# denix56/SI-Mamba

Hardware: AMD Instinct MI355X
Metric: point-clouds/sec (fwd+bwd) (higher is better)
Workload: dtype f32; 1 GPU; PointMamba classifier train step (FPS+kNN grouping, encoder, spectral SAST ordering, 12 Mamba blocks d=384 at L=1024, head, AdamW), 1024 pts -> 128 patches; global_batch=64, per_gpu_batch=64, npoints=1024, patches=128, mamba_seq_len=1024, parallelism=dp1, communicator_ranks=1, library_gemm=tuned solution table (si_mamba_amd/tuned/gemm_gfx950.csv)

## Files before the change

### si_mamba_amd/csrc/add_norm.hip

```cpp
#include "common.h"

namespace simamba {

constexpr int kLnThreads = 256;
constexpr int kLnMaxChunks = 8;

struct LnArgs {
  const void* hidden;
  const float* residual;
  const float* rowscale;
  const float* weight;
  const float* bias;
  float* residual_out;
  void* normed;
  float* mean;
  float* rstd;
  const void* dnormed;
  const float* dresidual_out;
  float* dresidual;
  void* dhidden;
  float* dwb_partial;
  const int* hidden_slot;
  const int* normed_slot;
  int hidden_batch, normed_batch;
  int batch, rows_per_batch, dim;
  float eps;
};

template <typename T>
__device__ __forceinline__ float4 ld4(const T* p) {
  const Pack<T, 4> pk = *reinterpret_cast<const Pack<T, 4>*>(p);
  return make_float4(to_f32<T>(pk.v[0]), to_f32<T>(pk.v[1]), to_f32<T>(pk.v[2]), to_f32<T>(pk.v[3]));
}
template <typename T>
__device__ __forceinline__ void st4(T* p, float4 v) {
  Pack<T, 4> pk;
  pk.v[0] = from_f32<T>(v.x); pk.v[1] = from_f32<T>(v.y); pk.v[2] = from_f32<T>(v.z); pk.v[3] = from_f32<T>(v.w);
  *reinterpret_cast<Pack<T, 4>*>(p) = pk;
}

__device__ __forceinline__ int ln_slot(const int* __restrict__ map, int b, int count) {
  if (!map) return b;
  const int s = __builtin_amdgcn_readfirstlane(map[b]);
  return (s >= 0 && s < count) ? s : -1;
}

struct LnRow {
  int b, hs, os;
};
__device__ __forceinline__ LnRow ln_row(const LnArgs& p, int row) {
  LnRow r;
  r.b = __builtin_amdgcn_readfirstlane(row / p.rows_per_batch);
  r.hs = ln_slot(p.hidden_slot, r.b, p.hidden_batch);
  r.os = ln_slot(p.normed_slot, r.b, p.normed_batch);
  return r;
}

template <typename TH, typename TO, int kChunks, bool kRms>
__global__ __launch_bounds__(kLnThreads) void add_ln_fwd_kernel(LnArgs p) {
  const bool slots = p.hidden_slot || p.normed_slot;
  const int lane = threadIdx.x & 63;
  const int wave_global = (blockIdx.x * kLnThreads + threadIdx.x) >> 6;
  const int nwaves = (gridDim.x * kLnThreads) >> 6;
  const int rows = p.batch * p.rows_per_batch;
  const int nch = p.dim >> 2;
  const TH* __restrict__ hg = static_cast<const TH*>(p.hidden);
  TO* __restrict__ og = static_cast<TO*>(p.normed);
  float4 w[kChunks], bs[kChunks];
#pragma unroll
  for (int k = 0; k < kChunks; ++k) {
    const int c = lane + 64 * k;
    w[k] = c < nch ? *reinterpret_cast<const float4*>(p.weight + 4 * c) : make_float4(0, 0, 0, 0);
    bs[k] = (!kRms && c < nch && p.bias) ? *reinterpret_cast<const float4*>(p.bias + 4 * c) : make_float4(0, 0, 0, 0);
  }
  const float inv_dim = 1.f / p.dim;
  LnRow next = (slots && wave_global < rows) ? ln_row(p, wave_global) : LnRow{0, 0, 0};
  for (int row = wave_global; row < rows; row += nwaves) {
    const size_t base = static_cast<size_t>(row) * p.dim;
    const float scale = (p.rowscale && p.residual) ? p.rowscale[row / p.rows_per_batch] : 1.f;
    size_t hbase = base, obase = base;
    bool has_h = true, has_o = true;
    if (slots) {
      const LnRow cur = next;
      const int ahead = row + nwaves;
      next = ln_row(p, ahead < rows ? ahead : row);
      const int r = __builtin_amdgcn_readfirstlane(row) - cur.b * p.rows_per_batch;
      has_h = cur.hs >= 0; has_o = cur.os >= 0;
      hbase = (static_cast<size_t>(has_h ? cur.hs : 0) * p.rows_per_batch + r) * p.dim;
      obase = (static_cast<size_t>(has_o ? cur.os : 0) * p.rows_per_batch + r) * p.dim;
    }
    float4 x[kChunks];
    float sum = 0.f;
#pragma unroll
    for (int k = 0; k < kChunks; ++k) {
      const int c = lane + 64 * k;
      if (c < nch) {
        float4 h;
        if (!has_h) {
          h = *reinterpret_cast<const float4*>(p.residual + base + 4 * c);
        } else {
          h = ld4<TH>(hg + hbase + 4 * c);
          if (p.residual) {
            const float4 r = *reinterpret_cast<const float4*>(p.residual + base + 4 * c);
            h.x = fmaf(h.x, scale, r.x); h.y = fmaf(h.y, scale, r.y);
            h.z = fmaf(h.z, scale, r.z); h.w = fmaf(h.w, scale, r.w);
          }
        }
        if (p.residual_out) *reinterpret_cast<float4*>(p.residual_out + base + 4 * c) = h;
        x[k] = h;
        sum += (h.x + h.y) + (h.z + h.w);
      } else {
        x[k] = make_float4(0, 0, 0, 0);
      }
    }
    if (!has_o) continue;
    const float mean = kRms ? 0.f : wave_allreduce_sum(sum) * inv_dim;
    float sq = 0.f;
#pragma unroll
    for (int k = 0; k < kChunks; ++k) {
      if (lane + 64 * k < nch) {
        const float a = x[k].x - mean, b = x[k].y - mean, c = x[k].z - mean, d = x[k].w - mean;
        sq += (a * a + b * b) + (c * c + d * d);
      }
    }
    const float rstd = rsqrtf(wave_allreduce_sum(sq) * inv_dim + p.eps);
#pragma unroll
    for (int k = 0; k < kChunks; ++k) {
      const int c = lane + 64 * k;
      if (c < nch) {
        float4 y;
        y.x = fmaf((x[k].x - mean) * rstd, w[k].x, bs[k].x);
        y.y = fmaf((x[k].y - mean) * rstd, w[k].y, bs[k].y);
        y.z = fmaf((x[k].z - mean) * rstd, w[k].z, bs[k].z);
        y.w = fmaf((x[k].w - mean) * rstd, w[k].w, bs[k].w);
        st4<TO>(og + obase + 4 * c, y);
      }
    }
    if (lane == 0) {
      if (!kRms) p.mean[row] = mean;
      p.rstd[row] = rstd;
    }
  }
}

template <typename TH, typename TO, int kChunks, bool kRms>
__global__ __launch_bounds__(kLnThreads) void add_ln_bwd_kernel(LnArgs p) {
  const bool slots = p.hidden_slot || p.normed_slot;
  extern __shared__ float sred[];
  const int lane = threadIdx.x & 63;
  const int wave = threadIdx.x >> 6;
  const int wave_global = (blockIdx.x * kLnThreads + threadIdx.x) >> 6;
  const int nwaves = (gridDim.x * kLnThreads) >> 6;
  const int rows = p.batch * p.rows_per_batch;
  const int nch = p.dim >> 2;
  const TO* __restrict__ dyg = static_cast<const TO*>(p.dnormed);
  TH* __restrict__ dhg = static_cast<TH*>(p.dhidden);
  float4 w[kChunks], dw[kChunks], db[kChunks];
#pragma unroll
  for (int k = 0; k < kChunks; ++k) {
    const int c = lane + 64 * k;
    w[k] = c < nch ? *reinterpret_cast<const float4*>(p.weight + 4 * c) : make_float4(0, 0, 0, 0);
    dw[k] = make_float4(0, 0, 0, 0);
    db[k] = make_float4(0, 0, 0, 0);
  }
  const float inv_dim = 1.f / p.dim;
  LnRow next = (slots && wave_global < rows) ? ln_row(p, wave_global) : LnRow{0, 0, 0};
  for (int row = wave_global; row < rows; row += nwaves) {
    const size_t base = static_cast<size_t>(row) * p.dim;
    size_t hbase = base, obase = base;
    bool has_h = true, has_o = true;
    if (slots) {
      const LnRow cur = next;
      const int ahead = row + nwaves;
      next = ln_row(p, ahead < rows ? ahead : row);
      const int r = __builtin_amdgcn_readfirstlane(row) - cur.b * p.rows_per_batch;
      has_h = cur.hs >= 0; has_o = cur.os >= 0;
      hbase = (static_cast<size_t>(has_h ? cur.hs : 0) * p.rows_per_batch + r) * p.dim;
      obase = (static_cast<size_t>(has_o ? cur.os : 0) * p.rows_per_batch + r) * p.dim;
    }
    if (!has_o) {
      const float scale = (p.rowscale && dhg) ? p.rowscale[row / p.rows_per_batch] : 1.f;
#pragma unroll
      for (int k = 0; k < kChunks; ++k) {
        const int c = lane + 64 * k;
        if (c < nch) {
          const float4 dx = p.dresidual_out ? *reinterpret_cast<const float4*>(p.dresidual_out + base + 4 * c)
                                            : make_float4(0, 0, 0, 0);
          if (p.dresidual) *reinterpret_cast<float4*>(p.dresidual + base + 4 * c) = dx;
          if (dhg && has_h)
            st4<TH>(dhg + hbase + 4 * c, make_float4(dx.x * scale, dx.y * scale, dx.z * scale, dx.w * scale));
        }
      }
      continue;
    }
    const float mean = kRms ? 0.f : p.mean[row], rstd = p.rstd[row];
    float4 xh[kChunks], g[kChunks];
    float s1 = 0.f, s2 = 0.f;
#pragma unroll
    for (int k = 0; k < kChunks; ++k) {
      const int c = lane + 64 * k;
      if (c < nch) {
        const float4 x = *reinterpret_cast<const float4*>(p.residual_out + base + 4 * c);
        const float4 dy = ld4<TO>(dyg + obase + 4 * c);
        xh[k] = make_float4((x.x - mean) * rstd, (x.y - mean) * rstd, (x.z - mean) * rstd, (x.w - mean) * rstd);
        g[k] = make_float4(dy.x * w[k].x, dy.y * w[k].y, dy.z * w[k].z, dy.w * w[k].w);
        dw[k].x = fmaf(dy.x, xh[k].x, dw[k].x); dw[k].y = fmaf(dy.y, xh[k].y, dw[k].y);
        dw[k].z = fmaf(dy.z, xh[k].z, dw[k].z); dw[k].w = fmaf(dy.w, xh[k].w, dw[k].w);
        db[k].x += dy.x; db[k].y += dy.y; db[k].z += dy.z; db[k].w += dy.w;
        s1 += (g[k].x + g[k].y) + (g[k].z + g[k].w);
        s2 += (g[k].x * xh[k].x + g[k].y * xh[k].y) + (g[k].z * xh[k].z + g[k].w * xh[k].w);
      } else {
        xh[k] = make_float4(0, 0, 0, 0);
        g[k] = make_float4(0, 0, 0, 0);
      }
    }
    const float c1 = kRms ? 0.f : wave_allreduce_sum(s1) * inv_dim;
    const float c2 = wave_allreduce_sum(s2) * inv_dim;
    const float scale = (p.rowscale && dhg) ? p.rowscale[row / p.rows_per_batch] : 1.f;
#pragma unroll
    for (int k = 0; k < kChunks; ++k) {
      const int c = lane + 64 * k;
      if (c < nch) {
        float4 dx;
        dx.x = (g[k].x - c1 - xh[k].x * c2) * rstd;
        dx.y = (g[k].y - c1 - xh[k].y * c2) * rstd;
        dx.z = (g[k].z - c1 - xh[k].z * c2) * rstd;
        dx.w = (g[k].w - c1 - xh[k].w * c2) * rstd;
        if (p.dresidual_out) {
          const float4 r = *reinterpret_cast<const float4*>(p.dresidual_out + base + 4 * c);
          dx.x += r.x; dx.y += r.y; dx.z += r.z; dx.w += r.w;
        }
        if (p.dresidual) *reinterpret_cast<float4*>(p.dresidual + base + 4 * c) = dx;
        if (dhg && has_h)
          st4<TH>(dhg + hbase + 4 * c, make_float4(dx.x * scale, dx.y * scale, dx.z * scale, dx.w * scale));
      }
    }
  }
  float* mine = sred + wave * 2 * p.dim;
#pragma unroll
  for (int k = 0; k < kChunks; ++k) {
    const int c = lane + 64 * k;
    if (c < nch) {
      *reinterpret_cast<float4*>(mine + 4 * c) = dw[k];
      if (!kRms) *reinterpret_cast<float4*>(mine + p.dim + 4 * c) = db[k];
    }
  }
  __syncthreads();
  float* out = p.dwb_partial + static_cast<size_t>(blockIdx.x) * 2 * p.dim;
  for (int i = threadIdx.x; i < (kRms ? 1 : 2) * p.dim; i += kLnThreads) {
    float v = 0.f;
#pragma unroll
    for (int wv = 0; wv < kLnThreads / 64; ++wv) v += sred[wv * 2 * p.dim + i];
    out[i] = v;
  }
}

static int ln_grid(int rows) {
  int g = (rows + 3) / 4;
  return g < 1 ? 1 : (g > 1024 ? 1024 : g);
}

template <typename TH, typename TO, bool kRms>
static int launch_ln(const LnArgs& a, bool bwd, int grid, hipStream_t s) {
  const int chunks = ((a.dim >> 2) + 63) / 64;
#define SIMAMBA_LN_CASE(K)                                                                                      \
  if (chunks <= K) {                                                                                             \
    if (bwd)                                                                                                     \
      hipLaunchKernelGGL((add_ln_bwd_kernel<TH, TO, K, kRms>), dim3(grid), dim3(kLnThreads),                     \
                         sizeof(float) * (kLnThreads / 64) * 2 * a.dim, s, a);                                   \
    else                                                                                                         \
      hipLaunchKernelGGL((add_ln_fwd_kernel<TH, TO, K, kRms>), dim3(grid), dim3(kLnThreads), 0, s, a);           \
    return static_cast<int>(hipGetLastError());                                                                  \
  }
  SIMAMBA_LN_CASE(1)
  SIMAMBA_LN_CASE(2)
  SIMAMBA_LN_CASE(4)
  SIMAMBA_LN_CASE(8)
#undef SIMAMBA_LN_CASE
  return SIMAMBA_E_SHAPE;
}

template <typename TH, typename TO>
static int launch_ln(const LnArgs& a, bool bwd, bool rms, int grid, hipStream_t s) {
  return rms ? launch_ln<TH, TO, true>(a, bwd, grid, s) : launch_ln<TH, TO, false>(a, bwd, grid, s);
}

static int dispatch_ln(const LnArgs& a, bool bwd, bool rms, int grid, int hidden_dtype, int out_dtype, hipStream_t s) {
  if (hidden_dtype == SIMAMBA_F32 && out_dtype == SIMAMBA_F32) return launch_ln<float, float>(a, bwd, rms, grid, s);
  if (hidden_dtype == SIMAMBA_BF16 && out_dtype == SIMAMBA_BF16)
    return launch_ln<bf16_t, bf16_t>(a, bwd, rms, grid, s);
  if (hidden_dtype == SIMAMBA_F32 && out_dtype == SIMAMBA_BF16) return launch_ln<float, bf16_t>(a, bwd, rms, grid, s);
  if (hidden_dtype == SIMAMBA_BF16 && out_dtype == SIMAMBA_F32) return launch_ln<bf16_t, float>(a, bwd, rms, grid, s);
  return SIMAMBA_E_DTYPE;
}

}

using namespace simamba;

static int check_ln(int batch, int rows_per_batch, int dim) {
  if (batch < 0 || rows_per_batch < 0) return SIMAMBA_E_SHAPE;
  if (dim <= 0 || (dim & 3) || dim > 64 * 4 * kLnMaxChunks) return SIMAMBA_E_SHAPE;
  return SIMAMBA_OK;
}

extern "C" int simamba_add_layer_norm_grid(int batch, int rows_per_batch) {
  const long long rows = static_cast<long long>(batch) * rows_per_batch;
  return ln_grid(rows > 2000000000ll ? 2000000000 : static_cast<int>(rows));
}

static int check_slots(const int* map, int compact_batch, int batch) {
  if (compact_batch < 0 || compact_batch > batch) return SIMAMBA_E_SHAPE;
  if (!map && compact_batch != batch) return SIMAMBA_E_NULLPTR;
  return SIMAMBA_OK;
}

extern "C" int simamba_add_layer_norm_check_slots(const int* slots_host, int batch, int compact_batch) {
  if (batch < 0 || compact_batch < 0 || compact_batch > batch) return SIMAMBA_E_SHAPE;
  if (batch == 0) return SIMAMBA_OK;
  if (!slots_host) return SIMAMBA_E_NULLPTR;
  for (int b = 0; b < batch; ++b) {
    const int s = slots_host[b];
    if (s < -1 || s >= compact_batch) return SIMAMBA_E_SHAPE;
    if (s < 0) continue;
    for (int c = 0; c < b; ++c)
      if (slots_host[c] == s) return SIMAMBA_E_SHAPE;
  }
  return SIMAMBA_OK;
}

extern "C" int simamba_add_layer_norm_fwd_slots(const void* hidden, const float* residual, const float* rowscale,
                                                const float* weight, const float* bias, float* residual_out,
                                                void* normed, float* mean, float* rstd, const int* hidden_slot,
                                                int hidden_batch, const int* normed_slot, int normed_batch, int batch,
                                                int rows_per_batch, int dim, float eps, int hidden_dtype,
                                                int out_dtype, int flags, void* stream) {
  if (flags & ~SIMAMBA_NORM_RMS) return SIMAMBA_E_VARIANT;
  const bool rms = (flags & SIMAMBA_NORM_RMS) != 0;
  if (rms && bias) return SIMAMBA_E_BIAS;
  int rc = check_ln(batch, rows_per_batch, dim);
  if (rc) return rc;
  if (batch == 0 || rows_per_batch == 0) return SIMAMBA_OK;
  if ((rc = check_slots(hidden_slot, hidden_batch, batch))) return rc;
  if ((rc = check_slots(normed_slot, normed_batch, batch))) return rc;
  if ((!hidden && hidden_batch) || !weight || (!normed && normed_batch) || (!mean && !rms) || !rstd)
    return SIMAMBA_E_NULLPTR;
  if (hidden_slot && (!residual || !residual_out)) return SIMAMBA_E_NULLPTR;
  LnArgs a{};
  a.hidden = hidden; a.residual = residual; a.rowscale = rowscale; a.weight = weight; a.bias = bias;
  a.residual_out = residual_out; a.normed = normed; a.mean = mean; a.rstd = rstd;
  a.hidden_slot = hidden_slot; a.normed_slot = normed_slot; a.hidden_batch = hidden_batch; a.normed_batch = normed_batch;
  a.batch = batch; a.rows_per_batch = rows_per_batch; a.dim = dim; a.eps = eps;
  return dispatch_ln(a, false, rms, simamba_add_layer_norm_grid(batch, rows_per_batch), hidden_dtype, out_dtype,
                     static_cast<hipStream_t>(stream));
}

extern "C" int simamba_add_layer_norm_fwd_ex(const void* hidden, const float* residual, const float* rowscale,
                                             const float* weight, const float* bias, float* residual_out, void* normed,
                                             float* mean, float* rstd, int batch, int rows_per_batch, int dim,
                                             float eps, int hidden_dtype, int out_dtype, int flags, void* stream) {
  return simamba_add_layer_norm_fwd_slots(hidden, residual, rowscale, weight, bias, residual_out, normed, mean, rstd,
                                          nullptr, batch, nullptr, batch, batch, rows_per_batch, dim, eps, hidden_dtype,
                                          out_dtype, flags, stream);
}

extern "C" int simamba_add_layer_norm_fwd(const void* hidden, const float* residual, const float* rowscale,
                                          const float* weight, const float* bias, float* residual_out, void* normed,
                                          float* mean, float* rstd, int batch, int rows_per_batch, int dim, float eps,
                                          int hidden_dtype, int out_dtype, void* stream) {
  return simamba_add_layer_norm_fwd_ex(hidden, residual, rowscale, weight, bias, residual_out, normed, mean, rstd,
                                       batch, rows_per_batch, dim, eps, hidden_dtype, out_dtype, 0, stream);
}

extern "C" int simamba_add_layer_norm_bwd_slots(const void* dnormed, const float* dresidual_out,
                                                const float* residual_out, const float* mean, const float* rstd,
                                                const float* weight, const float* rowscale, float* dresidual,
                                                void* dhidden, float* dwb_partial, const int* hidden_slot,
                                                int hidden_batch, const int* normed_slot, int normed_batch, int batch,
                                                int rows_per_batch, int dim, int hidden_dtype, int out_dtype,
                                                int flags, void* stream) {
  if (flags & ~SIMAMBA_NORM_RMS) return SIMAMBA_E_VARIANT;
  const bool rms = (flags & SIMAMBA_NORM_RMS) != 0;
  int rc = check_ln(batch, rows_per_batch, dim);
  if (rc) return rc;
  if (batch == 0 || rows_per_batch == 0) return SIMAMBA_OK;
  if ((rc = check_slots(hidden_slot, hidden_batch, batch))) return rc;
  if ((rc = check_slots(normed_slot, normed_batch, batch))) return rc;
  if (hidden_batch == 0) dhidden = nullptr;
  if ((!dnormed || !residual_out || (!mean && !rms) || !rstd) && normed_batch) return SIMAMBA_E_NULLPTR;
  if (!weight || !dwb_partial || (!dresidual && !dhidden)) return SIMAMBA_E_NULLPTR;
  LnArgs a{};
  a.dnormed = dnormed; a.dresidual_out = dresidual_out; a.residual_out = const_cast<float*>(residual_out);
  a.mean = const_cast<float*>(mean); a.rstd = const_cast<float*>(rstd); a.weight = weight; a.rowscale = rowscale;
  a.dresidual = dresidual; a.dhidden = dhidden; a.dwb_partial = dwb_partial;
  a.hidden_slot = hidden_slot; a.normed_slot = normed_slot; a.hidden_batch = hidden_batch; a.normed_batch = normed_batch;
  a.batch = batch; a.rows_per_batch = rows_per_batch; a.dim = dim;
  return dispatch_ln(a, true, rms, simamba_add_layer_norm_grid(batch, rows_per_batch), hidden_dtype, out_dtype,
                     static_cast<hipStream_t>(stream));
}

extern "C" int simamba_add_layer_norm_bwd_ex(const void* dnormed, const float* dresidual_out,
                                             const float* residual_out, const float* mean, const float* rstd,
                                             const float* weight, const float* rowscale, float* dresidual,
                                             void* dhidden, float* dwb_partial, int batch, int rows_per_batch, int dim,
                                             int hidden_dtype, int out_dtype, int flags, void* stream) {
  return simamba_add_layer_norm_bwd_slots(dnormed, dresidual_out, residual_out, mean, rstd, weight, rowscale, dresidual,
                                          dhidden, dwb_partial, nullptr, batch, nullptr, batch, batch, rows_per_batch,
                                          dim, hidden_dtype, out_dtype, flags, stream);
}

extern "C" int simamba_add_layer_norm_bwd(const void* dnormed, const float* dresidual_out, const float* residual_out,
                                          const float* mean, const float* rstd, const float* weight,
                                          const float* rowscale, float* dresidual, void* dhidden, float* dwb_partial,
                                          int batch, int rows_per_batch, int dim, int hidden_dtype, int out_dtype,
                                          void* stream) {
  return simamba_add_layer_norm_bwd_ex(dnormed, dresidual_out, residual_out, mean, rstd, weight, rowscale, dresidual,
                                       dhidden, dwb_partial, batch, rows_per_batch, dim, hidden_dtype, out_dtype, 0,
                                       stream);
}
```

Before: 1161 point-clouds/s.

## Preload slot maps into lanes and issue row loads unconditionally in add-LN kernels

The per-batch slot maps and rowscales are loaded once per wave into registers and fetched with readlane, instead of scalar global loads on every row. Row loads for hidden, residual, dy and x are issued up front without branches, using clamped offsets and a dummy pointer for absent rows. In the backward kernel the dresidual_out load is hoisted early when there are few chunks. The aim is to overlap memory latency and drop per-row dependent scalar loads, at the cost of higher register pressure and some wasted loads.

```diff
diff --git a/si_mamba_amd/csrc/add_norm.hip b/si_mamba_amd/csrc/add_norm.hip
--- a/si_mamba_amd/csrc/add_norm.hip
+++ b/si_mamba_amd/csrc/add_norm.hip
@@ -28,8 +28,7 @@
 };
 
 template <typename T>
-__device__ __forceinline__ float4 ld4(const T* p) {
-  const Pack<T, 4> pk = *reinterpret_cast<const Pack<T, 4>*>(p);
+__device__ __forceinline__ float4 unpack4(const Pack<T, 4>& pk) {
   return make_float4(to_f32<T>(pk.v[0]), to_f32<T>(pk.v[1]), to_f32<T>(pk.v[2]), to_f32<T>(pk.v[3]));
 }
 template <typename T>
@@ -41,71 +40,120 @@
 
 __device__ __forceinline__ int ln_slot(const int* __restrict__ map, int b, int count) {
   if (!map) return b;
-  const int s = __builtin_amdgcn_readfirstlane(map[b]);
+  const int s = map[b];
   return (s >= 0 && s < count) ? s : -1;
+}
+
+constexpr int kLnMapRegs = 2;
+struct LnSamples {
+  int hs[kLnMapRegs], os[kLnMapRegs];
+  float scale[kLnMapRegs];
+  bool resident;
+};
+__device__ __forceinline__ LnSamples ln_samples(const LnArgs& p, int lane, bool use_scale) {
+  LnSamples m;
+  m.resident = p.batch <= 64 * kLnMapRegs;
+#pragma unroll
+  for (int j = 0; j < kLnMapRegs; ++j) {
+    const int b = lane + 64 * j;
+    const bool in = m.resident && b < p.batch;
+    m.hs[j] = in ? ln_slot(p.hidden_slot, b, p.hidden_batch) : -1;
+    m.os[j] = in ? ln_slot(p.normed_slot, b, p.normed_batch) : -1;
+    m.scale[j] = (in && use_scale) ? p.rowscale[b] : 1.f;
+  }
+  return m;
 }
 
 struct LnRow {
   int b, hs, os;
+  float scale;
 };
-__device__ __forceinline__ LnRow ln_row(const LnArgs& p, int row) {
+__device__ __forceinline__ LnRow ln_row(const LnArgs& p, const LnSamples& m, bool use_scale, int row) {
   LnRow r;
   r.b = __builtin_amdgcn_readfirstlane(row / p.rows_per_batch);
-  r.hs = ln_slot(p.hidden_slot, r.b, p.hidden_batch);
-  r.os = ln_slot(p.normed_slot, r.b, p.normed_batch);
+  if (m.resident) {
+    int hs = m.hs[0], os = m.os[0];
+    float sc = m.scale[0];
+#pragma unroll
+    for (int j = 1; j < kLnMapRegs; ++j)
+      if ((r.b >> 6) == j) { hs = m.hs[j]; os = m.os[j]; sc = m.scale[j]; }
+    r.hs = __builtin_amdgcn_readlane(hs, r.b & 63);
+    r.os = __builtin_amdgcn_readlane(os, r.b & 63);
+    r.scale = __builtin_bit_cast(float, __builtin_amdgcn_readlane(__builtin_bit_cast(int, sc), r.b & 63));
+  } else {
+    r.hs = __builtin_amdgcn_readfirstlane(ln_slot(p.hidden_slot, r.b, p.hidden_batch));
+    r.os = __builtin_amdgcn_readfirstlane(ln_slot(p.normed_slot, r.b, p.normed_batch));
+    r.scale = use_scale ? __builtin_bit_cast(float, __builtin_amdgcn_readfirstlane(
+                              __builtin_bit_cast(int, p.rowscale[r.b])))
+                        : 1.f;
+  }
   return r;
+}
+
+__device__ __forceinline__ void ln_setup_loads_done() {
+  __builtin_amdgcn_s_waitcnt(0x0f70);
 }
 
 template <typename TH, typename TO, int kChunks, bool kRms>
 __global__ __launch_bounds__(kLnThreads) void add_ln_fwd_kernel(LnArgs p) {
-  const bool slots = p.hidden_slot || p.normed_slot;
   const int lane = threadIdx.x & 63;
-  const int wave_global = (blockIdx.x * kLnThreads + threadIdx.x) >> 6;
+  const int wave_global = __builtin_amdgcn_readfirstlane((blockIdx.x * kLnThreads + threadIdx.x) >> 6);
   const int nwaves = (gridDim.x * kLnThreads) >> 6;
   const int rows = p.batch * p.rows_per_batch;
   const int nch = p.dim >> 2;
   const TH* __restrict__ hg = static_cast<const TH*>(p.hidden);
   TO* __restrict__ og = static_cast<TO*>(p.normed);
   float4 w[kChunks], bs[kChunks];
+  int off[kChunks];
+  bool valid[kChunks];
 #pragma unroll
   for (int k = 0; k < kChunks; ++k) {
     const int c = lane + 64 * k;
+    valid[k] = c < nch;
+    off[k] = 4 * (valid[k] ? c : nch - 1);
     w[k] = c < nch ? *reinterpret_cast<const float4*>(p.weight + 4 * c) : make_float4(0, 0, 0, 0);
     bs[k] = (!kRms && c < nch && p.bias) ? *reinterpret_cast<const float4*>(p.bias + 4 * c) : make_float4(0, 0, 0, 0);
   }
   const float inv_dim = 1.f / p.dim;
-  LnRow next = (slots && wave_global < rows) ? ln_row(p, wave_global) : LnRow{0, 0, 0};
+  const bool use_scale = p.rowscale && p.residual;
+  const LnSamples samples = ln_samples(p, lane, use_scale);
+  ln_setup_loads_done();
+  LnRow next = wave_global < rows ? ln_row(p, samples, use_scale, wave_global) : LnRow{0, 0, 0, 1.f};
   for (int row = wave_global; row < rows; row += nwaves) {
+    const LnRow cur = next;
+    const int ahead = row + nwaves;
+    next = ln_row(p, samples, use_scale, ahead < rows ? ahead : row);
     const size_t base = static_cast<size_t>(row) * p.dim;
-    const float scale = (p.rowscale && p.residual) ? p.rowscale[row / p.rows_per_batch] : 1.f;
-    size_t hbase = base, obase = base;
-    bool has_h = true, has_o = true;
-    if (slots) {
-      const LnRow cur = next;
-      const int ahead = row + nwaves;
-      next = ln_row(p, ahead < rows ? ahead : row);
-      const int r = __builtin_amdgcn_readfirstlane(row) - cur.b * p.rows_per_batch;
-      has_h = cur.hs >= 0; has_o = cur.os >= 0;
-      hbase = (static_cast<size_t>(has_h ? cur.hs : 0) * p.rows_per_batch + r) * p.dim;
-      obase = (static_cast<size_t>(has_o ? cur.os : 0) * p.rows_per_batch + r) * p.dim;
+    const int r = row - cur.b * p.rows_per_batch;
+    const bool has_h = cur.hs >= 0, has_o = cur.os >= 0;
+    const float scale = cur.scale;
+    const TH* hrow = has_h ? hg + (static_cast<size_t>(cur.hs) * p.rows_per_batch + r) * p.dim
+                           : reinterpret_cast<const TH*>(p.weight);
+    const size_t obase = (static_cast<size_t>(has_o ? cur.os : 0) * p.rows_per_batch + r) * p.dim;
+    Pack<TH, 4> hraw[kChunks];
+    float4 res[kChunks];
+#pragma unroll
+    for (int k = 0; k < kChunks; ++k) hraw[k] = *reinterpret_cast<const Pack<TH, 4>*>(hrow + off[k]);
+    if (p.residual) {
+#pragma unroll
+      for (int k = 0; k < kChunks; ++k) res[k] = *reinterpret_cast<const float4*>(p.residual + base + off[k]);
     }
     float4 x[kChunks];
     float sum = 0.f;
 #pragma unroll
     for (int k = 0; k < kChunks; ++k) {
       const int c = lane + 64 * k;
-      if (c < nch) {
-        float4 h;
-        if (!has_h) {
-          h = *reinterpret_cast<const float4*>(p.residual + base + 4 * c);
+      float4 h = unpack4<TH>(hraw[k]);
+      if (p.residual) {
+        const float4 rr = res[k];
+        if (has_h) {
+          h.x = fmaf(h.x, scale, rr.x); h.y = fmaf(h.y, scale, rr.y);
+          h.z = fmaf(h.z, scale, rr.z); h.w = fmaf(h.w, scale, rr.w);
         } else {
-          h = ld4<TH>(hg + hbase + 4 * c);
-          if (p.residual) {
-            const float4 r = *reinterpret_cast<const float4*>(p.residual + base + 4 * c);
-            h.x = fmaf(h.x, scale, r.x); h.y = fmaf(h.y, scale, r.y);
-            h.z = fmaf(h.z, scale, r.z); h.w = fmaf(h.w, scale, r.w);
-          }
+          h = rr;
         }
+      }
+      if (valid[k]) {
         if (p.residual_out) *reinterpret_cast<float4*>(p.residual_out + base + 4 * c) = h;
         x[k] = h;
         sum += (h.x + h.y) + (h.z + h.w);
@@ -113,12 +161,11 @@
         x[k] = make_float4(0, 0, 0, 0);
       }
     }
-    if (!has_o) continue;
     const float mean = kRms ? 0.f : wave_allreduce_sum(sum) * inv_dim;
     float sq = 0.f;
 #pragma unroll
     for (int k = 0; k < kChunks; ++k) {
-      if (lane + 64 * k < nch) {
+      if (valid[k]) {
         const float a = x[k].x - mean, b = x[k].y - mean, c = x[k].z - mean, d = x[k].w - mean;
         sq += (a * a + b * b) + (c * c + d * d);
       }
@@ -127,7 +174,7 @@
 #pragma unroll
     for (int k = 0; k < kChunks; ++k) {
       const int c = lane + 64 * k;
-      if (c < nch) {
+      if (valid[k] && has_o) {
         float4 y;
         y.x = fmaf((x[k].x - mean) * rstd, w[k].x, bs[k].x);
         y.y = fmaf((x[k].y - mean) * rstd, w[k].y, bs[k].y);
@@ -136,7 +183,7 @@
         st4<TO>(og + obase + 4 * c, y);
       }
     }
-    if (lane == 0) {
+    if (lane == 0 && has_o) {
       if (!kRms) p.mean[row] = mean;
       p.rstd[row] = rstd;
     }
@@ -145,47 +192,69 @@
 
 template <typename TH, typename TO, int kChunks, bool kRms>
 __global__ __launch_bounds__(kLnThreads) void add_ln_bwd_kernel(LnArgs p) {
-  const bool slots = p.hidden_slot || p.normed_slot;
   extern __shared__ float sred[];
   const int lane = threadIdx.x & 63;
   const int wave = threadIdx.x >> 6;
-  const int wave_global = (blockIdx.x * kLnThreads + threadIdx.x) >> 6;
+  const int wave_global = __builtin_amdgcn_readfirstlane((blockIdx.x * kLnThreads + threadIdx.x) >> 6);
   const int nwaves = (gridDim.x * kLnThreads) >> 6;
   const int rows = p.batch * p.rows_per_batch;
   const int nch = p.dim >> 2;
   const TO* __restrict__ dyg = static_cast<const TO*>(p.dnormed);
   TH* __restrict__ dhg = static_cast<TH*>(p.dhidden);
+  constexpr bool kEarlyRes = kChunks <= 4;
   float4 w[kChunks], dw[kChunks], db[kChunks];
+  int off[kChunks];
+  bool valid[kChunks];
 #pragma unroll
   for (int k = 0; k < kChunks; ++k) {
     const int c = lane + 64 * k;
+    valid[k] = c < nch;
+    off[k] = 4 * (valid[k] ? c : nch - 1);
     w[k] = c < nch ? *reinterpret_cast<const float4*>(p.weight + 4 * c) : make_float4(0, 0, 0, 0);
     dw[k] = make_float4(0, 0, 0, 0);
     db[k] = make_float4(0, 0, 0, 0);
   }
   const float inv_dim = 1.f / p.dim;
-  LnRow next = (slots && wave_global < rows) ? ln_row(p, wave_global) : LnRow{0, 0, 0};
+  const bool use_scale = p.rowscale && dhg;
+  const LnSamples samples = ln_samples(p, lane, use_scale);
+  ln_setup_loads_done();
+  LnRow next = wave_global < rows ? ln_row(p, samples, use_scale, wave_global) : LnRow{0, 0, 0, 1.f};
   for (int row = wave_global; row < rows; row += nwaves) {
+    const LnRow cur = next;
+    const int ahead = row + nwaves;
+    next = ln_row(p, samples, use_scale, ahead < rows ? ahead : row);
     const size_t base = static_cast<size_t>(row) * p.dim;
-    size_t hbase = base, obase = base;
-    bool has_h = true, has_o = true;
-    if (slots) {
-      const LnRow cur = next;
-      const int ahead = row + nwaves;
-      next = ln_row(p, ahead < rows ? ahead : row);
-      const int r = __builtin_amdgcn_readfirstlane(row) - cur.b * p.rows_per_batch;
-      has_h = cur.hs >= 0; has_o = cur.os >= 0;
-      hbase = (static_cast<size_t>(has_h ? cur.hs : 0) * p.rows_per_batch + r) * p.dim;
-      obase = (static_cast<size_t>(has_o ? cur.os : 0) * p.rows_per_batch + r) * p.dim;
+    const int r = row - cur.b * p.rows_per_batch;
+    const bool has_h = cur.hs >= 0, has_o = cur.os >= 0;
+    const float scale = cur.scale;
+    const size_t hbase = (static_cast<size_t>(has_h ? cur.hs : 0) * p.rows_per_batch + r) * p.dim;
+    const float* xrow = has_o ? p.residual_out + base : p.weight;
+    const TO* dyrow = has_o ? dyg + (static_cast<size_t>(cur.os) * p.rows_per_batch + r) * p.dim
+                            : reinterpret_cast<const TO*>(p.weight);
+    const float* mrow = (has_o && !kRms) ? p.mean + row : p.weight;
+    const float* srow = has_o ? p.rstd + row : p.weight;
+    float4 xraw[kChunks], res[kChunks];
+    Pack<TO, 4> dyraw[kChunks];
+#pragma unroll
+    for (int k = 0; k < kChunks; ++k) {
+      xraw[k] = *reinterpret_cast<const float4*>(xrow + off[k]);
+      dyraw[k] = *reinterpret_cast<const Pack<TO, 4>*>(dyrow + off[k]);
+    }
+    const float mean_ld = *mrow, rstd = *srow;
+    if (kEarlyRes && p.dresidual_out) {
+#pragma unroll
+      for (int k = 0; k < kChunks; ++k) res[k] = *reinterpret_cast<const float4*>(p.dresidual_out + base + off[k]);
+    } else {
+#pragma unroll
+      for (int k = 0; k < kChunks; ++k) res[k] = make_float4(0, 0, 0, 0);
     }
     if (!has_o) {
-      const float scale = (p.rowscale && dhg) ? p.rowscale[row / p.rows_per_batch] : 1.f;
 #pragma unroll
       for (int k = 0; k < kChunks; ++k) {
         const int c = lane + 64 * k;
-        if (c < nch) {
-          const float4 dx = p.dresidual_out ? *reinterpret_cast<const float4*>(p.dresidual_out + base + 4 * c)
-                                            : make_float4(0, 0, 0, 0);
+        if (valid[k]) {
+          if (!kEarlyRes && p.dresidual_out) res[k] = *reinterpret_cast<const float4*>(p.dresidual_out + base + 4 * c);
+          const float4 dx = res[k];
           if (p.dresidual) *reinterpret_cast<float4*>(p.dresidual + base + 4 * c) = dx;
           if (dhg && has_h)
             st4<TH>(dhg + hbase + 4 * c, make_float4(dx.x * scale, dx.y * scale, dx.z * scale, dx.w * scale));
@@ -193,15 +262,14 @@
       }
       continue;
     }
-    const float mean = kRms ? 0.f : p.mean[row], rstd = p.rstd[row];
+    const float mean = kRms ? 0.f : mean_ld;
     float4 xh[kChunks], g[kChunks];
     float s1 = 0.f, s2 = 0.f;
 #pragma unroll
     for (int k = 0; k < kChunks; ++k) {
-      const int c = lane + 64 * k;
-      if (c < nch) {
-        const float4 x = *reinterpret_cast<const float4*>(p.residual_out + base + 4 * c);
-        const float4 dy = ld4<TO>(dyg + obase + 4 * c);
+      if (valid[k]) {
+        const float4 x = xraw[k];
+        const float4 dy = unpack4<TO>(dyraw[k]);
         xh[k] = make_float4((x.x - mean) * rstd, (x.y - mean) * rstd, (x.z - mean) * rstd, (x.w - mean) * rstd);
         g[k] = make_float4(dy.x * w[k].x, dy.y * w[k].y, dy.z * w[k].z, dy.w * w[k].w);
         dw[k].x = fmaf(dy.x, xh[k].x, dw[k].x); dw[k].y = fmaf(dy.y, xh[k].y, dw[k].y);
@@ -216,19 +284,20 @@
     }
     const float c1 = kRms ? 0.f : wave_allreduce_sum(s1) * inv_dim;
     const float c2 = wave_allreduce_sum(s2) * inv_dim;
-    const float scale = (p.rowscale && dhg) ? p.rowscale[row / p.rows_per_batch] : 1.f;
 #pragma unroll
     for (int k = 0; k < kChunks; ++k) {
       const int c = lane + 64 * k;
-      if (c < nch) {
+      if (valid[k]) {
         float4 dx;
         dx.x = (g[k].x - c1 - xh[k].x * c2) * rstd;
         dx.y = (g[k].y - c1 - xh[k].y * c2) * rstd;
         dx.z = (g[k].z - c1 - xh[k].z * c2) * rstd;
         dx.w = (g[k].w - c1 - xh[k].w * c2) * rstd;
+        if (!kEarlyRes && p.dresidual_out) res[k] = *reinterpret_cast<const float4*>(p.dresidual_out + base + 4 * c);
         if (p.dresidual_out) {
-          const float4 r = *reinterpret_cast<const float4*>(p.dresidual_out + base + 4 * c);
-          dx.x += r.x; dx.y += r.y; dx.z += r.z; dx.w += r.w;
+#pragma clang fp contract(off)
+          const float4 rr = res[k];
+          dx.x += rr.x; dx.y += rr.y; dx.z += rr.z; dx.w += rr.w;
         }
         if (p.dresidual) *reinterpret_cast<float4*>(p.dresidual + base + 4 * c) = dx;
         if (dhg && has_h)
```

Result: no change. 1170 point-clouds/s (median of 6 runs) (+0.7%).
